# eritpchy/video-subtitle-extractor

Hardware: AMD Instinct MI355X
Metric: OCR frames/sec (det+rec) @1080p (higher is better)
Workload: dtype f16

## Files before the change

include/vse_hip.h:

```cpp
#ifndef VSE_HIP_H
#define VSE_HIP_H

#include <stddef.h>
#include <stdint.h>

#ifdef __cplusplus
extern "C" {
#endif

#define VSE_OK 0
#define VSE_E_INVAL (-1)
#define VSE_E_HIP (-2)
#define VSE_E_UNSUPPORTED (-3)
#define VSE_E_NOMEM (-4)

typedef struct vse_ctx vse_ctx;
typedef struct vse_plan vse_plan;

#pragma pack(push, 1)
typedef struct vse_view {
    int64_t off;
    int32_t arena;
    int32_t n, h, w;
    int32_t c;
// ... 37 lines not shown
                    int64_t frame_stride, int dst_h, int dst_w, int raw_input, void* d_in_f16, float* d_prob, void* stream);
int vse_rec_forward(vse_ctx* ctx, vse_plan* rec_plan, void* ws, const void* d_rec_in_f16, const int32_t* d_widths, int out_level,
                    void* d_idx_maxp, int b, int t, int32_t* d_out_idx, int32_t* d_out_len, float* d_out_conf, void* stream);

typedef struct vse_graph vse_graph;
int vse_rec_graph_create(vse_ctx* ctx, vse_plan* rec_plan, void* ws, const void* d_rec_in_f16, const int32_t* d_widths, int out_level,
                         void* d_idx_maxp, int b, int t, int32_t* d_out_idx, int32_t* d_out_len, float* d_out_conf, void* stream,
                         vse_graph** graph);
int vse_graph_launch(vse_graph* graph, void* stream);
void vse_graph_destroy(vse_graph* graph);

int vse_plan_profile(vse_plan* plan, void* ws, void* const* ext, int n_ext, const int32_t* d_widths, void* stream, float* ms);

const char* vse_op_kernel_name(const vse_op* op);

int vse_det_preprocess(vse_ctx* ctx, const void* d_bgr, int n, int src_h, int src_w, int64_t pitch,
                       int64_t frame_stride, void* d_out_f16, int dst_h, int dst_w, const float* mean3,
                       const float* std3, void* stream);

typedef struct vse_db_params {
    double box_thresh;
    double unclip_ratio;
    float thresh;
    int max_candidates;
    int min_size;
} vse_db_params;

typedef struct vse_box {
    float pts[4][2];
    float score;
// ... 53 lines not shown
```

video-subtitle-extractor_amd/csrc/conv_c3.hip:

```cpp
#include "conv_common.h"
#ifdef VSE_TRACE
#include <stdio.h>
#include <vector>
#define TR_STAMP(i) do { if (tid == 0) tr[i] = __builtin_amdgcn_s_memtime(); } while (0)
#else
#define TR_STAMP(i) do { } while (0)
#endif

#define C3RING 4

template <int RW, int CW, int BN>
__device__ __forceinline__ void conv_c3_body(const ConvParams& p) {
    constexpr int TN = BN / 32;
    constexpr int TH = 2 * RW, TW = 32 * CW;
    constexpr int PW = TW + 8, PH = TH + 2;
    constexpr int PPIX = (PH * PW + 31) / 32 * 32;
    constexpr int PINSTR = PPIX / 32;
    constexpr int PNPL = (PINSTR + 7) / 8;
    constexpr int WROWS = 3 * BN;
    constexpr int WINSTR = WROWS / 32;
    constexpr int PATCH_HALFS = PPIX * 16, WSTAGE_HALFS = WROWS * 16;
    constexpr int PATCH_BYTES = PATCH_HALFS * 2, WSTAGE_BYTES = WSTAGE_HALFS * 2;
    constexpr int ROWB = PW * 32;
    static_assert(RW * CW == 8 && (PW / 8) % 2 == 1, "tile shapes");
    static_assert(2 * PATCH_BYTES + C3RING * WSTAGE_BYTES + 1024 + 4 * BN <= 81920, "two blocks per CU");
    __shared__ __attribute__((aligned(16))) half_t lds[2 * PATCH_HALFS + C3RING * WSTAGE_HALFS + 512 + 2 * BN];
// ... 12 lines not shown
#endif
    TR_STAMP(0);

    unsigned t = xcd_block(blockIdx.x, gridDim.x);
    const int nt = t % p.ntn;  t /= p.ntn;
    const int tx = t % p.tiles_w;  t /= p.tiles_w;
    const int ty = t % p.tiles_h;
    const int oy0 = ty * TH, ox0 = tx * TW, n0 = nt * BN;
    const ConvPackTile pk = conv_pack_tile(p, (int)(t / p.tiles_h), ox0, TW, 3);
    if (ox0 >= pk.vw) return;
    if (conv_tile_right_of_sample<TH, TW>(p, pk.img0, oy0, ox0, n0, BN)) return;
    const int nch1 = p.cinp >> 4;
    const int nchunks = (p.flags & F_HILO) ? 2 * nch1 : nch1;

    int poff[PNPL];
#pragma unroll
    for (int j = 0; j < PNPL; ++j) {
        const int q = 32 * (wave + 8 * j) + (lane >> 1);
        const int kh_ = (lane & 1) ^ ((q >> 3) & 1);
        const int py = q / PW, px = q - py * PW;
        const int iy = oy0 - 1 + py;
        int g, ix;
        const bool ok = conv_pack_src(p, pk, px, g, ix) && (py < PH) && (iy >= 0) && (iy < p.H);
        const long o = (((long)g * p.Hs + (iy >> p.inshift)) * p.Ws + (ix >> p.inshift)) * (long)p.in_ld + kh_ * 8;
        poff[j] = ok ? (int)o : -1;
    }
    const half_t* const in_img = p.in + pk.img0 * (long)p.Hs * p.Ws * p.in_ld;
    const half_t* wptr;
    bool wok;
    const int wnp = p.wnp;
    const int winc = 3 * wnp * 16;
    {
        const int row = 32 * wave + (lane >> 1);
        const int kh_ = (lane & 1) ^ ((row >> 3) & 1);
        const int dy = row / BN, r = row - dy * BN;
        wok = (row < WROWS) && (n0 + r < wnp);
        wptr = wok ? p.w + ((long)dy * wnp + n0 + r) * 16 + kh_ * 8 : p.zero;
    }
    auto issue_patch = [&](int cc) {
        half_t* base = patch0 + (cc & 1) * PATCH_HALFS;
        const bool live = cc < nchunks;
#pragma unroll
        for (int j = 0; j < PNPL; ++j) {
            const int i = wave + 8 * j;
            const half_t* src = (live && poff[j] >= 0) ? in_img + poff[j] + (cc >= nch1 ? cc - nch1 : cc) * 16 : p.zero;
            half_t* dst = base + i * 512;
            if (i >= PINSTR) { src = p.zero; dst = dummy0; }
            glds16_asm(src, dst);
        }
    };
    auto issue_w = [&](int s) {
        half_t* st = ring0 + (s & (C3RING - 1)) * WSTAGE_HALFS;
        glds16_asm(wptr, wave < WINSTR ? st + wave * 512 : dummy0);
        wptr += wok ? winc : 0;
    };

// ... 144 lines not shown
    }
#ifdef VSE_TRACE
    asm volatile("s_waitcnt vmcnt(0)" ::: "memory");
    if (tid == 0 && p.trace) {
        tr[3] = __builtin_amdgcn_s_memtime();
        tr[4] = t_sync;
        for (int i = 0; i < 8; ++i) p.trace[(unsigned long long)blockIdx.x * 8 + i] = tr[i];
    }
#endif
}

template <int RW, int CW>
__global__ __launch_bounds__(512, 4) void conv_c3_kernel(const ConvParams p) { conv_c3_body<RW, CW, C3BN>(p); }
template <int RW, int CW>
__global__ __launch_bounds__(512, 4) void conv_c3n32_kernel(const ConvParams p) { conv_c3_body<RW, CW, 32>(p); }

static const ConvInst kC3Inst[] = {
    CONV_INST(8, 1, 0, conv_c3n32_kernel<8, 1>), CONV_INST(4, 1, 0, conv_c3n32_kernel<4, 2>), CONV_INST(2, 1, 0, conv_c3n32_kernel<2, 4>),
    CONV_INST(8, 0, 0, conv_c3_kernel<8, 1>),    CONV_INST(4, 0, 0, conv_c3_kernel<4, 2>),    CONV_INST(2, 0, 0, conv_c3_kernel<2, 4>),
};

static int launch_conv_c3(const ConvParams& pin, const ConvKernel& k, hipStream_t st) {
    const ConvInst* inst = conv_inst(conv_c3_family(), k);
    if (!inst) return VSE_E_UNSUPPORTED;
    ConvParams p = pin;
    const int rw = k.arg[0], cw = 8 / rw;
    conv_pack_plan(p, 32 * cw, 6);
    if ((double)p.pack_g * p.Hs * p.Ws * p.in_ld > 2.0e9) conv_pack_plan(p, 32 * cw, -1);
    if ((double)p.Hs * p.Ws * p.in_ld > 2.0e9) return VSE_E_UNSUPPORTED;
    const bool hlsum = (p.flags & F_HLSUM) != 0;
    if (hlsum && (p.Np > 32 || (p.flags & F_HILO))) return VSE_E_INVAL;
    const int bn = k.arg[1] ? 32 : C3BN;
    p.wnp = hlsum ? 64 : p.Np;
    p.ntn = hlsum ? 1u : (unsigned)((p.Np + bn - 1) / bn);
    p.tiles_h = (p.OH + 2 * rw - 1) / (2 * rw);
    const unsigned long long blocks = (unsigned long long)((p.nimg + p.pack_g - 1) / p.pack_g) * p.tiles_h * p.tiles_w * p.ntn;
    if (blocks == 0 || blocks > 0x7fffffffull) return VSE_E_INVAL;
    const dim3 grid((unsigned)blocks), block(512);
#ifdef VSE_TRACE
    static unsigned long long* trace_dev = nullptr;
    static size_t trace_cap = 0;
    if (trace_cap < blocks * 8) {
        if (trace_dev) (void)hipFree(trace_dev);
        (void)hipMalloc(&trace_dev, blocks * 8 * sizeof(unsigned long long));
        trace_cap = blocks * 8;
// ... 26 lines not shown
```

video-subtitle-extractor_amd/csrc/conv_common.h:

```cpp
#pragma once
#include "common.h"

#define PTW 32
#define CTW 32
#define CPW 48
#define C3BN 64
#define PW_MAXN 256
#define PW_MAXN_HILO 128
#define DWPW_ROWS_MAX_KS 3
#define DWPW_ROWS_MAX_KS_S1 3

struct ConvParams {
    const half_t* in;
    const half_t* w;
    const float* bias;
    const half_t* res;
    const half_t* zero;
    void* out;
    int H, W, Hs, Ws, in_ld, cinp, inshift;
    int OH, OW;
    long M;
    int kh, kw, sh, sw, ph, pw;
    int Np, nk;
    int nkh;
// ... 18 lines not shown
    const int* wl_out;
    int in_lo_off;
    int res_lo_off;
    int lo_off;
    const half_t* ogate;
    int ogate_ld;
    int wnp;
    const uint8_t* u8src;
    int u8_h, u8_w;
    long u8_pitch, u8_fstride;
    int pack_g, nimg;
    unsigned pack_mag_ow, pack_mag_d;
    int pool_seg, pool_nseg;
};

typedef const __attribute__((address_space(1))) void* gptr_t;
typedef __attribute__((address_space(3))) void* lptr_t;

__device__ __forceinline__ void glds16(const void* g, half_t* l) {
    __builtin_amdgcn_global_load_lds((gptr_t)g, (lptr_t)l, 16, 0, 0);
}

__device__ __forceinline__ void glds16_asm(const void* g, half_t* l) {
    unsigned keep;
    const unsigned dst = __builtin_amdgcn_readfirstlane((unsigned)(size_t)(lptr_t)l);
    asm volatile("s_mov_b32 %0, m0\n\ts_mov_b32 m0, %2\n\ts_nop 0\n\tglobal_load_lds_dwordx4 %1, off\n\ts_mov_b32 m0, %0"
                 : "=&s"(keep) : "v"(g), "s"(dst) : "memory");
}

#define OOB 0x80000000u
// ... 245 lines not shown

struct GemmCfg { int bm, bn, wm, wn, bk, st; };
constexpr GemmCfg kCfg[] = {{128, 128, 2, 2, 32, 3}, {256, 64, 4, 1, 32, 3}, {256, 32, 4, 1, 32, 3}, {256, 128, 4, 2, 32, 3},
                            {256, 256, 4, 4, 32, 3}, {256, 192, 8, 2, 32, 3}, {256, 256, 4, 4, 64, 2}, {256, 192, 8, 2, 64, 2}};

struct SrcGeom { int h, w; long pitch, fstride; };
ConvParams conv_params(const vse_op& o, const TView& in, const TView& res, const TView& in2, const TView& out, const TView& dot_out,
                       const char* wts, const half_t* zero, const int* wl_out, const uint8_t* u8src, const SrcGeom& src);
ConvKernel conv_select(const ConvParams& p, int Kp);
int conv_kernel_name(const ConvKernel& k, char* buf, size_t n);
int launch_conv(const vse_op& o, const TView& in, const TView& res, const TView& in2, const TView& out, const TView& dot_out,
                const char* wts, const half_t* zero, const int* wl_out, const uint8_t* u8src, const SrcGeom& src, hipStream_t st);
ConvKernel conv_pool_select(const vse_op* ops, int n_ops, int i);
int launch_conv_pool(const vse_op& conv, const ConvKernel& k, const TView& in, const TView& pool_out, const char* wts, const half_t* zero,
                     hipStream_t st);
static inline long conv_images(const ConvParams& p) { return p.OH && p.OW ? p.M / ((long)p.OH * p.OW) : 0; }
int conv_pack_group(long images, int OW, int TW, int spare, int gap);
void conv_pack_plan(ConvParams& p, int TW, int spare);
```

video-subtitle-extractor_amd/csrc/conv_select.hip:

```cpp
#include <stdlib.h>
#include <cstdio>
#include "conv_common.h"


static int conv_gemm_mode(int kh, int kw, int sh, int sw, int ph, int pw, int cinp, int Kp, int inshift, int flags) {
    (void)sh; (void)sw;
    if (inshift || (flags & (F_PATCH | F_DOT1 | F_SRC2))) return 0;
    if (cinp % 32) return 0;
    if (kh * kw > 31) return 0;
    if (kh < 2 * ph + 1 || kw < 2 * pw) return 0;
    if (kh == 1 && kw == 1 && ph == 0 && pw == 0 && Kp == cinp) return 2;
    return 1;
}
static bool conv_gemm_span_ok(const ConvParams& p, int Kp) {
    const double span = ((double)512 * p.sw + (512.0 / p.OW + 3) * p.sh * p.Ws + (double)p.kh * p.Ws + p.kw) * p.in_ld * 2;
    return !(span > 1.9e9 || (double)Kp * p.Np * 2 > 1.9e9);
}

static int conv_gemm_config(int Np, int cinp, long M) {
    auto ntn = [&](int bn) { return (long)((Np + bn - 1) / bn); };
    auto deep = [&](int c) { return cinp % 64 == 0 ? c + 2 : c; };
    if (Np <= 32) return 2;
    if (Np <= 64) return 1;
    const long mt = (M + 255) / 256;
// ... 296 lines not shown
}

int launch_conv_pool(const vse_op& conv, const ConvKernel& k, const TView& in, const TView& pool_out, const char* wts, const half_t* zero,
                     hipStream_t st) {
    if (k.family != CK_C3POOL || !in.ptr || !pool_out.ptr || !zero) return VSE_E_INVAL;
    const TView none{nullptr, 0, 0, 0, 0, 0, 0};
    const TView shape{nullptr, conv.out.n, conv.out.h, conv.out.w, conv.out.c, conv.out.ld, conv.out.esize};
    ConvParams p = conv_params(conv, in, none, none, shape, none, wts, zero, nullptr, nullptr, SrcGeom{0, 0, 0, 0});
    if (in.c != p.cinp || (in.ld & 7)) return VSE_E_INVAL;
    p.out = pool_out.ptr;
    p.out_ld = pool_out.ld;
    return conv_launch(p, k, st);
}


int launch_conv(const vse_op& o, const TView& in, const TView& res, const TView& in2, const TView& out, const TView& dot_out,
                const char* wts, const half_t* zero, const int* wl_out, const uint8_t* u8src, const SrcGeom& src, hipStream_t st) {
    const ConvParams p = conv_params(o, in, res, in2, out, dot_out, wts, zero, wl_out, u8src, src);
    const int f = p.flags, Np = p.Np, cinp = p.cinp;
    if (f & F_SRC2) {
        if (!in2.ptr || in2.esize != 2 || (in2.ld & 7) || in.c + in2.c != cinp) return VSE_E_INVAL;
        if ((in2.h << p.in2_shift) != p.H || (in2.w << p.in2_shift) != p.W) return VSE_E_INVAL;
    } else if (in.c != cinp) {
        return VSE_E_INVAL;
    }
    if (in.esize != 2 || ((in.ld & 7) && !((f & F_UP2HEAD) && in.ld == 1)) || (cinp & 7)) return VSE_E_INVAL;
    if ((f & F_RES) && (res.esize != 2 || (res.ld & 3))) return VSE_E_INVAL;
    if ((!(f & (F_DOT1 | F_ONECH)) && (out.ld & 3)) || (Np & 7)) return VSE_E_INVAL;
    if ((f & F_ONECH) && (!(f & F_PIXSHUF) || !(f & F_OUT_F32) || Np != 32 || out.ld != 1 || out.esize != 4 || (f & F_RES)))
        return VSE_E_INVAL;
// ... 16 lines not shown
```

video-subtitle-extractor_amd/csrc/vse_runtime.hip:

```cpp
#include <stdlib.h>
#include <cstdarg>
#include <cstdio>
#include <cstring>
#include <string>
#include <vector>

#include "conv_common.h"

static thread_local std::string g_err;
static void set_err(const char* fmt, ...) {
    char buf[512];
    va_list ap;
    va_start(ap, fmt);
    vsnprintf(buf, sizeof buf, fmt, ap);
    va_end(ap);
    g_err = buf;
}
void vse_set_error(const char* msg) { g_err = msg ? msg : ""; }
#define HIP_TRY(expr)                                                                  \
    do {                                                                               \
        hipError_t e_ = (expr);                                                        \
        if (e_ != hipSuccess) {                                                        \
            set_err("%s failed: %s (%s:%d)", #expr, hipGetErrorString(e_), __FILE__, __LINE__); \
            return VSE_E_HIP;                                                          \
        }                                                                              \
    } while (0)

struct vse_ctx {
    int device;
    std::vector<void*> weights;
    std::vector<size_t> weight_bytes;
    void* zero_page;
};

struct vse_plan {
    vse_ctx* ctx;
    int weights_id;
    std::vector<vse_op> ops;
    std::vector<ConvKernel> pooled;
    size_t ws_bytes;
    int max_ext;
    int n_levels;
    int batch;
    bool u8_source;
    int src_h, src_w;
    long src_pitch, src_fstride;
};

int vse_frame_change_launch(const void* d_bgr, int n, int64_t pitch, int64_t frame_stride, int y0, int y1, int x0, int x1, int edge_thresh,
                            void* d_state, int reset, int32_t* d_counts, void* stream);
int vse_scene_change_plane_pitch(int aw);
int vse_scene_change_launch(const void* d_bgr, int n, int64_t pitch, int64_t frame_stride, int scale, int ah, int aw, int search, int bias,
                            void* d_state, int reset, void* d_ws, int32_t* d_counts, void* stream);
size_t vse_audio_match_ws(const long* m, const long* n, int nq);
int vse_audio_match_launch(const uint8_t* const* pat, const uint8_t* const* win, const long* m, const long* n, int nq, void* d_ws,
                           unsigned long long* d_out, void* stream);

extern "C" {

const char* vse_last_error(void) { return g_err.c_str(); }
size_t vse_sizeof_op(void) { return sizeof(vse_op); }
size_t vse_sizeof_view(void) { return sizeof(vse_view); }
int vse_abi_version(void) { return 4; }

int vse_init(int device_id, vse_ctx** out) {
    if (!out) return VSE_E_INVAL;
    int count = 0;
    HIP_TRY(hipGetDeviceCount(&count));
    if (device_id < 0 || device_id >= count) {
        set_err("device %d not present (%d visible)", device_id, count);
        return VSE_E_INVAL;
// ... 109 lines not shown
                set_err("op %d: chain descriptor out of the weight blob", i);
                delete p;
                return VSE_E_INVAL;
            }
            if (hdr[0] != 0x43484e31 || hdr[1] != o.p[3] || hdr[2] != o.p[4] || hdr[5] != o.p[2] || hdr[3] < 0 || hdr[4] < 0 ||
                (size_t)o.w_off + (size_t)hdr[4] + (size_t)hdr[3] > wbytes) {
                set_err("op %d: chain descriptor does not match its record (magic %#x, stages %d / %d, buffers %d / %d, LDS %d / %d)", i, hdr[0],
                        hdr[1], o.p[3], hdr[2], o.p[4], hdr[5], o.p[2]);
                delete p;
                return VSE_E_INVAL;
            }
        }
    }
    p->pooled.assign(n_ops, ConvKernel{CK_NONE, VSE_OK, {0, 0, 0}});
    for (int i = 0; i + 1 < n_ops && !p->n_levels; ++i) p->pooled[i] = conv_pool_select(ops, n_ops, i);
    *out = p;
    return VSE_OK;
}

void vse_plan_destroy(vse_plan* p) { delete p; }

static inline TView resolve(const vse_view& v, char* ws, char* wts, void* const* ext) {
    TView t;
    t.ptr = nullptr;
    t.n = v.n; t.h = v.h; t.w = v.w; t.c = v.c; t.ld = v.ld; t.esize = v.esize;
    if (v.n == 0) return t;
    char* base = v.arena == 0 ? ws : (v.arena == 1 ? wts : reinterpret_cast<char*>(ext[v.arena - 2]));
    t.ptr = base + v.off;
    return t;
}

static int run_op(vse_plan* p, int i, char* ws, void* const* ext, const int32_t* wtab, hipStream_t st, const SrcGeom& src) {
    const vse_op& o = p->ops[i];
    const int* wl_in = (wtab && o.p[P_WLIN]) ? wtab + (size_t)(o.p[P_WLIN] - 1) * p->batch : nullptr;
    const int* wl_out = (wtab && o.p[P_WLOUT]) ? wtab + (size_t)(o.p[P_WLOUT] - 1) * p->batch : nullptr;
    char* wts = reinterpret_cast<char*>(p->ctx->weights[p->weights_id]);
    const TView in0 = resolve(o.in0, ws, wts, ext), in1 = resolve(o.in1, ws, wts, ext),
                in2 = resolve(o.in2, ws, wts, ext), out = resolve(o.out, ws, wts, ext),
                out2 = resolve(o.out2, ws, wts, ext);
    int rc;
    if (i > 0 && p->pooled[i - 1].family == CK_C3POOL) return VSE_OK;
    if (p->pooled[i].family == CK_C3POOL) {
        const TView pool_out = resolve(p->ops[i + 1].out, ws, wts, ext);
        rc = launch_conv_pool(o, p->pooled[i], in0, pool_out, wts, reinterpret_cast<const half_t*>(p->ctx->zero_page), st);
    } else if (o.kind == OP_CONV) {
        const uint8_t* u8src = (o.flags & F_U8SRC) ? reinterpret_cast<const uint8_t*>(ext[0]) : nullptr;
        rc = launch_conv(o, in0, in1, in2, out, out2, wts, reinterpret_cast<const half_t*>(p->ctx->zero_page), wl_out, u8src, src, st);
    } else if (o.kind == OP_CHAIN) {
        rc = launch_chain(o, in0, out, out2, in2, wts, st);
    } else {
        rc = launch_simple_op(o, in0, in1, in2, out, out2, wts, wl_in, wl_out, st);
    }
    if (rc != VSE_OK) set_err("op %d (kind %d) failed to launch: rc=%d (%s)", i, o.kind, rc, hipGetErrorString(hipGetLastError()));
    return rc;
}

static int check_run(vse_plan* p, void* ws, void* const* ext, int n_ext, const int32_t* d_widths, const char* who) {
// ... 288 lines not shown
    if (rc0 != VSE_OK) return rc0;
    hipStream_t st = reinterpret_cast<hipStream_t>(stream);
    const int n = (int)p->ops.size();
    std::vector<hipEvent_t> ev(n + 1);
    for (auto& e : ev) HIP_TRY(hipEventCreate(&e));
    HIP_TRY(hipEventRecord(ev[0], st));
    for (int i = 0; i < n; ++i) {
        int rc = run_op(p, i, reinterpret_cast<char*>(ws), ext, d_widths, st, SrcGeom{p->src_h, p->src_w, p->src_pitch, p->src_fstride});
        if (rc != VSE_OK) return rc;
        HIP_TRY(hipEventRecord(ev[i + 1], st));
    }
    HIP_TRY(hipStreamSynchronize(st));
    for (int i = 0; i < n; ++i) HIP_TRY(hipEventElapsedTime(&ms[i], ev[i], ev[i + 1]));
    for (int i = 1; i < n; ++i)
        if (p->pooled[i - 1].family == CK_C3POOL) ms[i] = 0.f;
    for (auto& e : ev) (void)hipEventDestroy(e);
    return VSE_OK;
}

}
```

video-subtitle-extractor_amd/engine.py:

```python
import ctypes as C
import os

import numpy as np

from . import compiler, ir

_HERE = os.path.dirname(os.path.abspath(__file__))
LIB_PATH = os.environ.get("VSE_LIB_PATH") or os.path.join(_HERE, "libvse_hip.so")

EXPORTS = [
    "vse_init", "vse_destroy", "vse_last_error", "vse_sizeof_op", "vse_sizeof_view", "vse_abi_version",
    "vse_weights_upload", "vse_weights_free", "vse_plan_create", "vse_plan_destroy", "vse_plan_run", "vse_plan_run_ragged",
    "vse_plan_width_levels", "vse_plan_profile", "vse_op_kernel_name", "vse_det_preprocess", "vse_db_workspace_bytes",
    "vse_db_postprocess", "vse_rec_preprocess", "vse_rec_preprocess_scratch_bytes", "vse_ctc_collapse", "vse_ctc_collapse_ragged",
    "vse_det_forward", "vse_rec_forward", "vse_plan_set_source", "vse_plan_takes_frames",
    "vse_rec_graph_create", "vse_graph_launch", "vse_graph_destroy", "vse_frame_change_state_bytes", "vse_frame_change",
    "vse_audio_match_workspace_bytes", "vse_audio_match", "vse_scene_change_state_bytes", "vse_scene_change_workspace_bytes",
    "vse_scene_change",
]


class VseError(RuntimeError):
    pass


class DbParams(C.Structure):
    _fields_ = [("box_thresh", C.c_double), ("unclip_ratio", C.c_double), ("thresh", C.c_float),
                ("max_candidates", C.c_int), ("min_size", C.c_int)]


class Box(C.Structure):
    _fields_ = [("pts", C.c_float * 2 * 4), ("score", C.c_float), ("frame", C.c_int)]

# ... 45 lines not shown
    lib.vse_rec_graph_create.argtypes = [C.c_void_p, C.c_void_p, C.c_void_p, C.c_void_p, C.c_void_p, C.c_int, C.c_void_p, C.c_int, C.c_int,
                                         C.c_void_p, C.c_void_p, C.c_void_p, C.c_void_p, C.POINTER(C.c_void_p)]
    lib.vse_graph_launch.argtypes = [C.c_void_p, C.c_void_p]
    lib.vse_graph_destroy.argtypes = [C.c_void_p]
    lib.vse_graph_destroy.restype = None
    lib.vse_plan_set_source.argtypes = [C.c_void_p, C.c_int, C.c_int, C.c_int64, C.c_int64]
    lib.vse_plan_takes_frames.argtypes = [C.c_void_p]
    lib.vse_det_forward.argtypes = [C.c_void_p, C.c_void_p, C.c_void_p, C.c_void_p, C.c_int, C.c_int, C.c_int, C.c_int64, C.c_int64,
                                    C.c_int, C.c_int, C.c_int, C.c_void_p, C.c_void_p, C.c_void_p]
    lib.vse_rec_forward.argtypes = [C.c_void_p, C.c_void_p, C.c_void_p, C.c_void_p, C.c_void_p, C.c_int, C.c_void_p, C.c_int, C.c_int,
                                    C.c_void_p, C.c_void_p, C.c_void_p, C.c_void_p]
    lib.vse_plan_profile.argtypes = [C.c_void_p, C.c_void_p, C.POINTER(C.c_void_p), C.c_int, C.c_void_p, C.c_void_p,
                                     C.POINTER(C.c_float)]
    lib.vse_op_kernel_name.argtypes = [C.c_void_p]
    lib.vse_op_kernel_name.restype = C.c_char_p
    lib.vse_det_preprocess.argtypes = [C.c_void_p, C.c_void_p, C.c_int, C.c_int, C.c_int, C.c_int64, C.c_int64,
                                       C.c_void_p, C.c_int, C.c_int, C.POINTER(C.c_float), C.POINTER(C.c_float),
                                       C.c_void_p]
    lib.vse_db_postprocess.argtypes = [C.c_void_p, C.c_void_p, C.c_int, C.c_int, C.c_int, C.c_int, C.c_int,
                                       C.POINTER(DbParams), C.c_void_p, C.c_size_t, C.POINTER(Box), C.c_int,
                                       C.POINTER(C.c_int), C.c_void_p]
    lib.vse_rec_preprocess.argtypes = [C.c_void_p, C.c_void_p, C.c_int, C.c_int, C.c_int, C.c_int64, C.c_int64,
                                       C.POINTER(Crop), C.c_int, C.c_void_p, C.c_int, C.c_int, C.c_void_p,
                                       C.c_size_t, C.c_void_p]
    lib.vse_ctc_collapse.argtypes = [C.c_void_p, C.c_void_p, C.c_int, C.c_int, C.c_void_p, C.c_void_p, C.c_void_p,
                                     C.c_void_p]
    lib.vse_ctc_collapse_ragged.argtypes = [C.c_void_p, C.c_void_p, C.c_int, C.c_int, C.c_void_p, C.c_void_p, C.c_void_p,
                                            C.c_void_p, C.c_void_p]
    lib.vse_frame_change_state_bytes.restype = C.c_size_t
    lib.vse_frame_change_state_bytes.argtypes = [C.c_int, C.c_int]
# ... 4 lines not shown
    lib.vse_audio_match.argtypes = [C.c_void_p, C.c_void_p, C.c_int64, C.c_void_p, C.c_int64, C.c_void_p, C.c_int, C.c_void_p,
                                    C.c_size_t, C.c_void_p, C.c_void_p]
    lib.vse_scene_change_state_bytes.restype = C.c_size_t
    lib.vse_scene_change_state_bytes.argtypes = [C.c_int, C.c_int, C.c_int]
    lib.vse_scene_change_workspace_bytes.restype = C.c_size_t
    lib.vse_scene_change_workspace_bytes.argtypes = [C.c_int, C.c_int, C.c_int, C.c_int]
    lib.vse_scene_change.argtypes = [C.c_void_p, C.c_void_p, C.c_int, C.c_int, C.c_int, C.c_int64, C.c_int64, C.c_int, C.c_int, C.c_int,
                                     C.c_void_p, C.c_int, C.c_void_p, C.c_size_t, C.c_void_p, C.c_void_p]
    if lib.vse_sizeof_op() != ir.OP_DT.itemsize or lib.vse_sizeof_view() != ir.VIEW_DT.itemsize:
        raise VseError(f"ABI mismatch: vse_op {lib.vse_sizeof_op()} vs {ir.OP_DT.itemsize}, "
                       f"vse_view {lib.vse_sizeof_view()} vs {ir.VIEW_DT.itemsize}")
    _lib = lib
    return lib


def op_kernel_names(ops):
    lib = load_library()
    ops = np.ascontiguousarray(ops)
    base = ops.ctypes.data
    return [lib.vse_op_kernel_name(C.c_void_p(base + i * ops.itemsize)).decode() for i in range(len(ops))]


def profiled_kernel_names(ops, ms):
    names = op_kernel_names(ops)
    for i in range(1, len(names)):
        if (int(ops[i]["kind"]) == ir.OP_POOL and int(ops[i - 1]["kind"]) == ir.OP_CONV and float(ms[i]) == 0.0
                and names[i - 1].startswith("conv_patch_kernel<")):
            names[i - 1] = "conv_c3pool_kernel<%s>" % names[i - 1].split(",")[1].strip()
    return names


def _check(rc, what):
    if rc < 0:
        raise VseError(f"{what} failed (rc={rc}): {load_library().vse_last_error().decode(errors='replace')}")
    return rc


def _torch():
    import torch
    if not torch.cuda.is_available():
        raise VseError("no HIP device visible: the OCR hot path runs only on MI355X (gfx950); no CPU fallback")
    return torch


# ... 389 lines not shown
    def profile_frames(self, frames_u8, dst_h, dst_w, slot=0):
        if not self.fuse_preprocess:
            return self.profile(self.ctx.det_preprocess(frames_u8, dst_h, dst_w, raw=self.input_norm is not None), slot)
        t = self.ctx.torch
        n, h, w, _ = frames_u8.shape
        self.program(n, dst_h, dst_w)
        prog, handle = self._ensure((n, dst_h, dst_w))
        _check(self.ctx.lib.vse_plan_set_source(handle, h, w, frames_u8.stride(1), frames_u8.stride(0)), "vse_plan_set_source")
        outs = [t.empty((o["n"], o["h"], o["w"], o["ld"]), dtype=t.float32, device=self.ctx.tdev) for o in prog.outputs]
        ptrs = (C.c_void_p * (1 + len(outs)))(frames_u8.data_ptr(), *[o.data_ptr() for o in outs])
        ms = (C.c_float * len(prog.ops))()
        ws = self._workspace((n, dst_h, dst_w), prog, slot)
        self.last_outs = outs
        _check(self.ctx.lib.vse_plan_profile(handle, C.c_void_p(ws.data_ptr()), ptrs, len(ptrs), None, self.ctx.stream(), ms),
               "vse_plan_profile")
        names = profiled_kernel_names(prog.ops, ms)
        return np.array(ms[:], dtype=np.float32), prog, names

    def rec_forward(self, x, widths=None, slot=0):
        t = self.ctx.torch
        assert x.dtype == t.float16 and x.is_contiguous() and x.shape[3] == 8
        n, h, w, _ = x.shape
        self.program(n, h, w)
        prog, handle = self._ensure((n, h, w))
        assert len(prog.outputs) == 1 and prog.outputs[0]["kind"] == "idx_maxp"
        tt = prog.outputs[0]["w"]
        wt = self._width_table(prog, widths, n, w)
        idx_maxp = t.empty((n, 1, tt, 2), dtype=t.float32, device=self.ctx.tdev)
        oi = t.zeros((n, tt), dtype=t.int32, device=self.ctx.tdev)
        ol = t.empty((n,), dtype=t.int32, device=self.ctx.tdev)
        oc = t.empty((n,), dtype=t.float32, device=self.ctx.tdev)
# ... 41 lines not shown
        return bufs["oi"].clone(), bufs["ol"].clone(), bufs["oc"].clone()

    def profile(self, x, slot=0, widths=None):
        n, h, w, _ = x.shape
        self.program(n, h, w)
        prog, handle = self._ensure((n, h, w))
        outs, ptrs = self._ext(prog, x)
        ms = (C.c_float * len(prog.ops))()
        ws = self._workspace((n, h, w), prog, slot)
        wt = self._width_table(prog, widths, n, w)
        self.last_tlen = wt[prog.out_level] if wt is not None else None
        self.last_outs = outs
        _check(self.ctx.lib.vse_plan_profile(handle, C.c_void_p(ws.data_ptr()), ptrs, len(ptrs),
                                             C.c_void_p(wt.data_ptr()) if wt is not None else None, self.ctx.stream(), ms),
               "vse_plan_profile")
        variants = profiled_kernel_names(prog.ops, ms)
        return np.array(ms[:], dtype=np.float32), prog, variants
```

Measured before the change: 2097.

## Fuse channel-concat resizes into 3x3 conv via multi-part gather input table

Adds a gather variant of the c3 3x3 conv kernel that reads its input channels from up to four source tensors (with per-part upsample shift), driven by a small device-side part table. The plan detects convs whose input is a concat written by resize ops and absorbs those resizes, skipping their launches and the intermediate concat write and read. When a source would be overwritten before the conv, the resize is kept as a plain copy. The cost is extra per-chunk part switching and address recomputation inside the conv, plus extra plan analysis logic.

```diff
diff --git a/include/vse_hip.h b/include/vse_hip.h
--- a/include/vse_hip.h
+++ b/include/vse_hip.h
@@ -75,6 +75,10 @@
 
 const char* vse_op_kernel_name(const vse_op* op);
 
+const char* vse_plan_kernel_name(vse_plan* plan, int i);
+int vse_plan_set_concat_gather(vse_plan* plan, int mode);
+int vse_concat_gather_parts(const vse_op* ops, int n_ops, int i, int32_t* info);
+
 int vse_det_preprocess(vse_ctx* ctx, const void* d_bgr, int n, int src_h, int src_w, int64_t pitch,
                        int64_t frame_stride, void* d_out_f16, int dst_h, int dst_w, const float* mean3,
                        const float* std3, void* stream);
diff --git a/video-subtitle-extractor_amd/csrc/conv_c3.hip b/video-subtitle-extractor_amd/csrc/conv_c3.hip
--- a/video-subtitle-extractor_amd/csrc/conv_c3.hip
+++ b/video-subtitle-extractor_amd/csrc/conv_c3.hip
@@ -9,7 +9,7 @@
 
 #define C3RING 4
 
-template <int RW, int CW, int BN>
+template <int RW, int CW, int BN, bool GATHER = false>
 __device__ __forceinline__ void conv_c3_body(const ConvParams& p) {
     constexpr int TN = BN / 32;
     constexpr int TH = 2 * RW, TW = 32 * CW;
@@ -52,18 +52,47 @@
     const int nchunks = (p.flags & F_HILO) ? 2 * nch1 : nch1;
 
     int poff[PNPL];
-#pragma unroll
-    for (int j = 0; j < PNPL; ++j) {
-        const int q = 32 * (wave + 8 * j) + (lane >> 1);
-        const int kh_ = (lane & 1) ^ ((q >> 3) & 1);
-        const int py = q / PW, px = q - py * PW;
-        const int iy = oy0 - 1 + py;
-        int g, ix;
-        const bool ok = conv_pack_src(p, pk, px, g, ix) && (py < PH) && (iy >= 0) && (iy < p.H);
-        const long o = (((long)g * p.Hs + (iy >> p.inshift)) * p.Ws + (ix >> p.inshift)) * (long)p.in_ld + kh_ * 8;
-        poff[j] = ok ? (int)o : -1;
-    }
-    const half_t* const in_img = p.in + pk.img0 * (long)p.Hs * p.Ws * p.in_ld;
+    const half_t* in_img;
+    int part_i = 0, part_next = 0x7fffffff;
+    auto load_part = [&](int pi) __attribute__((always_inline)) {
+        typedef const __attribute__((address_space(4))) ConvPart* cpart_t;
+        const cpart_t tab = reinterpret_cast<cpart_t>(reinterpret_cast<uintptr_t>(p.in2));
+        pi = __builtin_amdgcn_readfirstlane(pi);
+        ConvPart e;
+        e.off = tab[pi].off; e.ld = tab[pi].ld; e.shift = tab[pi].shift; e.c0 = tab[pi].c0; e.h = tab[pi].h; e.w = tab[pi].w;
+        part_i = pi;
+        part_next = pi + 1 < p.in2_ld ? tab[pi + 1].c0 >> 4 : 0x7fffffff;
+        in_img = p.in + e.off + pk.img0 * (long)e.h * e.w * e.ld - e.c0;
+        int ln = lane;
+        asm volatile("" : "+v"(ln));
+#pragma unroll
+        for (int j = 0; j < PNPL; ++j) {
+            const int q = 32 * (wave + 8 * j) + (ln >> 1);
+            const int kh_ = (ln & 1) ^ ((q >> 3) & 1);
+            const int py = q / PW, px = q - py * PW;
+            const int iy = oy0 - 1 + py;
+            int g, ix;
+            const bool ok = conv_pack_src(p, pk, px, g, ix) && (py < PH) && (iy >= 0) && (iy < p.H);
+            const long o = (((long)g * e.h + (iy >> e.shift)) * e.w + (ix >> e.shift)) * (long)e.ld + kh_ * 8;
+            poff[j] = ok ? (int)o : -1;
+        }
+    };
+    if constexpr (GATHER) {
+        load_part(0);
+    } else {
+#pragma unroll
+        for (int j = 0; j < PNPL; ++j) {
+            const int q = 32 * (wave + 8 * j) + (lane >> 1);
+            const int kh_ = (lane & 1) ^ ((q >> 3) & 1);
+            const int py = q / PW, px = q - py * PW;
+            const int iy = oy0 - 1 + py;
+            int g, ix;
+            const bool ok = conv_pack_src(p, pk, px, g, ix) && (py < PH) && (iy >= 0) && (iy < p.H);
+            const long o = (((long)g * p.Hs + (iy >> p.inshift)) * p.Ws + (ix >> p.inshift)) * (long)p.in_ld + kh_ * 8;
+            poff[j] = ok ? (int)o : -1;
+        }
+        in_img = p.in + pk.img0 * (long)p.Hs * p.Ws * p.in_ld;
+    }
     const half_t* wptr;
     bool wok;
     const int wnp = p.wnp;
@@ -78,6 +107,9 @@
     auto issue_patch = [&](int cc) {
         half_t* base = patch0 + (cc & 1) * PATCH_HALFS;
         const bool live = cc < nchunks;
+        if constexpr (GATHER) {
+            if (cc == part_next) load_part(part_i + 1);
+        }
 #pragma unroll
         for (int j = 0; j < PNPL; ++j) {
             const int i = wave + 8 * j;
@@ -252,10 +284,17 @@
 __global__ __launch_bounds__(512, 4) void conv_c3_kernel(const ConvParams p) { conv_c3_body<RW, CW, C3BN>(p); }
 template <int RW, int CW>
 __global__ __launch_bounds__(512, 4) void conv_c3n32_kernel(const ConvParams p) { conv_c3_body<RW, CW, 32>(p); }
+template <int RW, int CW>
+__global__ __launch_bounds__(512, 4) void conv_c3_gather_kernel(const ConvParams p) { conv_c3_body<RW, CW, C3BN, true>(p); }
+template <int RW, int CW>
+__global__ __launch_bounds__(512, 4) void conv_c3n32_gather_kernel(const ConvParams p) { conv_c3_body<RW, CW, 32, true>(p); }
 
 static const ConvInst kC3Inst[] = {
     CONV_INST(8, 1, 0, conv_c3n32_kernel<8, 1>), CONV_INST(4, 1, 0, conv_c3n32_kernel<4, 2>), CONV_INST(2, 1, 0, conv_c3n32_kernel<2, 4>),
     CONV_INST(8, 0, 0, conv_c3_kernel<8, 1>),    CONV_INST(4, 0, 0, conv_c3_kernel<4, 2>),    CONV_INST(2, 0, 0, conv_c3_kernel<2, 4>),
+    CONV_INST(8, 1, 1, conv_c3n32_gather_kernel<8, 1>), CONV_INST(4, 1, 1, conv_c3n32_gather_kernel<4, 2>),
+    CONV_INST(2, 1, 1, conv_c3n32_gather_kernel<2, 4>), CONV_INST(8, 0, 1, conv_c3_gather_kernel<8, 1>),
+    CONV_INST(4, 0, 1, conv_c3_gather_kernel<4, 2>),    CONV_INST(2, 0, 1, conv_c3_gather_kernel<2, 4>),
 };
 
 static int launch_conv_c3(const ConvParams& pin, const ConvKernel& k, hipStream_t st) {
@@ -267,6 +306,8 @@
     if ((double)p.pack_g * p.Hs * p.Ws * p.in_ld > 2.0e9) conv_pack_plan(p, 32 * cw, -1);
     if ((double)p.Hs * p.Ws * p.in_ld > 2.0e9) return VSE_E_UNSUPPORTED;
     const bool hlsum = (p.flags & F_HLSUM) != 0;
+    if (k.arg[2] && (!p.in2 || p.in2_ld < 1 || p.in2_ld > CONV_MAX_PARTS || p.inshift || p.wl_out || (p.flags & (F_HILO | F_HLSUM | F_SRC2))))
+        return VSE_E_INVAL;
     if (hlsum && (p.Np > 32 || (p.flags & F_HILO))) return VSE_E_INVAL;
     const int bn = k.arg[1] ? 32 : C3BN;
     p.wnp = hlsum ? 64 : p.Np;
diff --git a/video-subtitle-extractor_amd/csrc/conv_common.h b/video-subtitle-extractor_amd/csrc/conv_common.h
--- a/video-subtitle-extractor_amd/csrc/conv_common.h
+++ b/video-subtitle-extractor_amd/csrc/conv_common.h
@@ -56,6 +56,12 @@
     int pool_seg, pool_nseg;
 };
 
+#define CONV_MAX_PARTS 4
+struct ConvPart {
+    long off;
+    int ld, shift, c0, h, w, pad_;
+};
+
 typedef const __attribute__((address_space(1))) void* gptr_t;
 typedef __attribute__((address_space(3))) void* lptr_t;
 
@@ -331,6 +337,21 @@
 ConvKernel conv_pool_select(const vse_op* ops, int n_ops, int i);
 int launch_conv_pool(const vse_op& conv, const ConvKernel& k, const TView& in, const TView& pool_out, const char* wts, const half_t* zero,
                      hipStream_t st);
+struct ConvConcat {
+    int nparts;
+    struct {
+        vse_view src;
+        vse_view copy_from;
+        int shift, c0;
+        int writer;
+        int absorbed;
+    } part[CONV_MAX_PARTS];
+};
+ConvKernel conv_concat_select(const vse_op* ops, int n_ops, int i, ConvConcat* cc = nullptr);
+void conv_concat_table(const vse_op& conv, const ConvConcat& cc, ConvPart* tab);
+void conv_concat_force_copy(const vse_op& conv, ConvConcat& cc);
+int launch_conv_gather(const vse_op& conv, const ConvKernel& k, const TView& in, const TView& res, const TView& out, const char* wts,
+                       const half_t* zero, const ConvPart* d_tab, int nparts, hipStream_t st);
 static inline long conv_images(const ConvParams& p) { return p.OH && p.OW ? p.M / ((long)p.OH * p.OW) : 0; }
 int conv_pack_group(long images, int OW, int TW, int spare, int gap);
 void conv_pack_plan(ConvParams& p, int TW, int spare);
diff --git a/video-subtitle-extractor_amd/csrc/conv_select.hip b/video-subtitle-extractor_amd/csrc/conv_select.hip
--- a/video-subtitle-extractor_amd/csrc/conv_select.hip
+++ b/video-subtitle-extractor_amd/csrc/conv_select.hip
@@ -334,6 +334,137 @@
 }
 
 
+static bool channel_slice(const vse_view& w, const vse_view& v, int* c0) {
+    if (w.n == 0 || w.arena != v.arena || w.n != v.n || w.h != v.h || w.w != v.w || w.ld != v.ld || w.esize != v.esize) return false;
+    const int64_t d = w.off - v.off;
+    if (d < 0 || d % v.esize || d / v.esize + w.c > v.c) return false;
+    *c0 = (int)(d / v.esize);
+    return true;
+}
+static bool touches(const vse_op& o, const vse_view& v) {
+    return views_overlap(o.in0, v) || views_overlap(o.in1, v) || views_overlap(o.in2, v) || views_overlap(o.out, v) || views_overlap(o.out2, v);
+}
+static bool reads(const vse_op& o, const vse_view& v) {
+    return views_overlap(o.in0, v) || views_overlap(o.in1, v) || (o.kind != OP_CHAIN && views_overlap(o.in2, v)) ||
+           (o.kind != OP_CONV && o.kind != OP_CHAIN && views_overlap(o.out2, v));
+}
+static bool writes(const vse_op& o, const vse_view& v) {
+    return views_overlap(o.out, v) || ((o.kind == OP_CONV || o.kind == OP_CHAIN) && views_overlap(o.out2, v)) ||
+           (o.kind == OP_CHAIN && views_overlap(o.in2, v));
+}
+static void part_to_copy(const vse_view& V, ConvConcat& t, int q) {
+    auto& e = t.part[q];
+    if (!e.absorbed || e.copy_from.n) return;
+    e.copy_from = e.src;
+    e.src.off = V.off + (int64_t)e.c0 * V.esize;
+    e.src.arena = V.arena;
+    e.src.ld = V.ld;
+}
+void conv_concat_force_copy(const vse_op& conv, ConvConcat& cc) {
+    for (int q = 0; q < cc.nparts; ++q) part_to_copy(conv.in0, cc, q);
+}
+
+ConvKernel conv_concat_select(const vse_op* ops, int n_ops, int i, ConvConcat* cc) {
+    const ConvKernel no{CK_NONE, VSE_OK, {0, 0, 0}};
+    if (!ops || i < 1 || i >= n_ops) return no;
+    const vse_op& c = ops[i];
+    if (c.kind != OP_CONV || (c.flags & ~(F_COL | F_RES)) || !(c.flags & F_COL)) return no;
+    if (c.p[P_KH] != 3 || c.p[P_KW] != 3 || c.p[P_SH] != 1 || c.p[P_SW] != 1 || c.p[P_PH] != 1 || c.p[P_PW] != 1) return no;
+    if (c.p[P_INSHIFT] || c.p[P_LO_OUT] || c.p[P_LO_RES] || c.p[P_WLIN] || c.p[P_WLOUT] || c.in2.n || c.out2.n) return no;
+    const vse_view& V = c.in0;
+    if (V.n == 0 || V.arena != 0 || V.esize != 2 || V.c != c.p[P_CINP] || (V.ld & 7) || (V.off & 15)) return no;
+    auto shape = [](const vse_view& v) { return TView{nullptr, v.n, v.h, v.w, v.c, v.ld, v.esize}; };
+    const ConvParams prm = conv_params(c, shape(c.in0), shape(c.in1), shape(c.in2), shape(c.out), shape(c.out2), nullptr, nullptr, nullptr, nullptr,
+                                       SrcGeom{0, 0, 0, 0});
+    const ConvKernel k = conv_select(prm, c.p[P_KTOT]);
+    if (k.family != CK_C3 || k.rc != VSE_OK || k.arg[2]) return no;
+
+    ConvConcat t{};
+    int covered = 0, first = i;
+    auto add = [&](const vse_view& src, const vse_view& from, int shift, int c0, int ch, int writer) {
+        if (t.nparts == CONV_MAX_PARTS || (c0 & 15) || (ch & 15) || ch <= 0) return false;
+        for (int q = 0; q < t.nparts; ++q)
+            if (c0 < t.part[q].c0 + t.part[q].src.c && t.part[q].c0 < c0 + ch) return false;
+        auto& e = t.part[t.nparts++];
+        e.src = src; e.src.c = ch; e.copy_from = from; e.shift = shift; e.c0 = c0; e.writer = writer;
+        covered += ch;
+        return true;
+    };
+    auto source_ok = [&](const vse_view& sv, int shift, int ch) {
+        return sv.n == V.n && sv.arena == 0 && sv.esize == 2 && sv.c >= ch && !(sv.ld & 7) && !(sv.off & 15) && shift >= 0 && shift <= 3 &&
+               (sv.h << shift) == V.h && (sv.w << shift) == V.w && !views_overlap(sv, V);
+    };
+    for (int j = i - 1; j >= 0 && covered < V.c; --j) {
+        const vse_op& o = ops[j];
+        int c0;
+        if (!channel_slice(o.out, V, &c0)) {
+            if (touches(o, V)) return no;
+            continue;
+        }
+        if (views_overlap(o.in0, V) || views_overlap(o.in1, V) || views_overlap(o.in2, V) || views_overlap(o.out2, V)) return no;
+        if (o.p[P_WLIN] || o.p[P_WLOUT]) return no;
+        first = j;
+        if (o.kind == OP_CONV) {
+            if (o.p[P_LO_OUT] || (o.flags & (F_PIXSHUF | F_OUT_F32 | F_DOT1 | F_ONECH)) || o.out.c != o.p[P_COUT]) return no;
+            if (!add(o.out, vse_view{}, 0, c0, o.out.c, j)) return no;
+        } else if (o.kind == OP_RESIZE && !(o.flags & F_GATE) && !(o.flags & ~(F_SRC2 | F_RES))) {
+            const bool two = (o.flags & F_SRC2) != 0;
+            const int ca = two ? o.in0.c : o.out.c, cb = two ? o.in2.c : 0;
+            if (o.in1.n || o.out2.n || (!two && o.in2.n) || ca + cb != o.out.c) return no;
+            if (!source_ok(o.in0, o.p[0], ca) || !add(o.in0, vse_view{}, o.p[0], c0, ca, j)) return no;
+            if (two && (!source_ok(o.in2, o.p[1], cb) || !add(o.in2, vse_view{}, o.p[1], c0 + ca, cb, j))) return no;
+        } else {
+            return no;
+        }
+    }
+    if (covered != V.c || t.nparts < 2) return no;
+    bool any = false;
+    for (int q = 0; q < t.nparts; ++q) any = any || ops[t.part[q].writer].kind == OP_RESIZE;
+    if (!any) return no;
+    (void)first;
+    for (int j = i + 1; j < n_ops; ++j) {
+        const vse_op& o = ops[j];
+        if (reads(o, V)) return no;
+        if (writes(o, V)) break;
+    }
+    for (int a = 0; a < t.nparts; ++a)
+        for (int b = a + 1; b < t.nparts; ++b)
+            if (t.part[b].c0 < t.part[a].c0) { const auto x = t.part[a]; t.part[a] = t.part[b]; t.part[b] = x; }
+    for (int q = 0; q < t.nparts; ++q) {
+        auto& e = t.part[q];
+        if (ops[e.writer].kind != OP_RESIZE) continue;
+        e.absorbed = 1;
+        bool lives = !views_overlap(c.out, e.src) && !views_overlap(c.out2, e.src);
+        for (int j = e.writer + 1; j < i && lives; ++j) lives = !writes(ops[j], e.src);
+        if (!lives) part_to_copy(V, t, q);
+    }
+    for (int q = 0; q < t.nparts; ++q)
+        if (16.0 * t.part[q].src.h * t.part[q].src.w * (t.part[q].src.ld > V.ld ? t.part[q].src.ld : V.ld) > 2.0e9) return no;
+    if (cc) *cc = t;
+    return ConvKernel{CK_C3, VSE_OK, {k.arg[0], k.arg[1], 1}};
+}
+
+void conv_concat_table(const vse_op& conv, const ConvConcat& cc, ConvPart* tab) {
+    for (int q = 0; q < cc.nparts; ++q) {
+        const auto& e = cc.part[q];
+        tab[q] = ConvPart{(e.src.off - conv.in0.off) / 2, e.src.ld, e.shift, e.c0, e.src.h, e.src.w, 0};
+    }
+}
+
+int launch_conv_gather(const vse_op& conv, const ConvKernel& k, const TView& in, const TView& res, const TView& out, const char* wts,
+                       const half_t* zero, const ConvPart* d_tab, int nparts, hipStream_t st) {
+    if (k.family != CK_C3 || !k.arg[2] || !in.ptr || !out.ptr || !zero || !d_tab) return VSE_E_INVAL;
+    const TView none{nullptr, 0, 0, 0, 0, 0, 0};
+    ConvParams p = conv_params(conv, in, res, none, out, none, wts, zero, nullptr, nullptr, SrcGeom{0, 0, 0, 0});
+    if (in.c != p.cinp || in.esize != 2 || (in.ld & 7) || (p.cinp & 15) || (out.ld & 3) || (p.Np & 7)) return VSE_E_INVAL;
+    if ((p.flags & F_RES) && (res.esize != 2 || (res.ld & 3))) return VSE_E_INVAL;
+    if (out.h != p.OH || out.w != p.OW || out.n != in.n) return VSE_E_INVAL;
+    p.in2 = reinterpret_cast<const half_t*>(d_tab);
+    p.in2_ld = nparts;
+    return conv_launch(p, k, st);
+}
+
+
 int launch_conv(const vse_op& o, const TView& in, const TView& res, const TView& in2, const TView& out, const TView& dot_out,
                 const char* wts, const half_t* zero, const int* wl_out, const uint8_t* u8src, const SrcGeom& src, hipStream_t st) {
     const ConvParams p = conv_params(o, in, res, in2, out, dot_out, wts, zero, wl_out, u8src, src);
diff --git a/video-subtitle-extractor_amd/csrc/vse_runtime.hip b/video-subtitle-extractor_amd/csrc/vse_runtime.hip
--- a/video-subtitle-extractor_amd/csrc/vse_runtime.hip
+++ b/video-subtitle-extractor_amd/csrc/vse_runtime.hip
@@ -38,6 +38,12 @@
     int weights_id;
     std::vector<vse_op> ops;
     std::vector<ConvKernel> pooled;
+    std::vector<ConvKernel> gathered;
+    std::vector<ConvConcat> parts;
+    std::vector<int> gather_slot;
+    std::vector<char> absorbed;
+    std::vector<std::vector<std::pair<vse_view, vse_view>>> copies;
+    ConvPart* d_parts;
     size_t ws_bytes;
     int max_ext;
     int n_levels;
@@ -55,6 +61,8 @@
 size_t vse_audio_match_ws(const long* m, const long* n, int nq);
 int vse_audio_match_launch(const uint8_t* const* pat, const uint8_t* const* win, const long* m, const long* n, int nq, void* d_ws,
                            unsigned long long* d_out, void* stream);
+
+static int plan_concat_commit(vse_plan* p);
 
 extern "C" {
 
@@ -194,11 +202,97 @@
     }
     p->pooled.assign(n_ops, ConvKernel{CK_NONE, VSE_OK, {0, 0, 0}});
     for (int i = 0; i + 1 < n_ops && !p->n_levels; ++i) p->pooled[i] = conv_pool_select(ops, n_ops, i);
+    p->gathered.assign(n_ops, ConvKernel{CK_NONE, VSE_OK, {0, 0, 0}});
+    p->parts.assign(n_ops, ConvConcat{});
+    p->gather_slot.assign(n_ops, -1);
+    p->absorbed.assign(n_ops, 0);
+    p->copies.assign(n_ops, {});
+    p->d_parts = nullptr;
+    for (int i = 0; i < n_ops && !p->n_levels; ++i) {
+        ConvConcat cc;
+        const ConvKernel k = conv_concat_select(ops, n_ops, i, &cc);
+        if (k.family != CK_C3) continue;
+        bool taken = false;
+        for (int j = 0; j < i; ++j)
+            for (int q = 0; q < cc.nparts && p->gathered[j].family == CK_C3; ++q)
+                for (int r = 0; r < p->parts[j].nparts; ++r) taken = taken || (cc.part[q].absorbed && p->parts[j].part[r].writer == cc.part[q].writer);
+        if (taken) continue;
+        p->gathered[i] = k;
+        p->parts[i] = cc;
+    }
+    if (plan_concat_commit(p) != VSE_OK) {
+        if (p->d_parts) (void)hipFree(p->d_parts);
+        delete p;
+        return VSE_E_HIP;
+    }
     *out = p;
     return VSE_OK;
 }
 
-void vse_plan_destroy(vse_plan* p) { delete p; }
+void vse_plan_destroy(vse_plan* p) {
+    if (p && p->d_parts) (void)hipFree(p->d_parts);
+    delete p;
+}
+
+static int plan_concat_commit(vse_plan* p) {
+    const int n = (int)p->ops.size();
+    p->absorbed.assign(n, 0);
+    p->copies.assign(n, {});
+    std::vector<ConvPart> tabs;
+    for (int i = 0; i < n; ++i) {
+        p->gather_slot[i] = -1;
+        if (p->gathered[i].family != CK_C3) continue;
+        p->gather_slot[i] = (int)tabs.size() / CONV_MAX_PARTS;
+        tabs.resize(tabs.size() + CONV_MAX_PARTS, ConvPart{});
+        conv_concat_table(p->ops[i], p->parts[i], &tabs[tabs.size() - CONV_MAX_PARTS]);
+        for (int q = 0; q < p->parts[i].nparts; ++q) {
+            const auto& e = p->parts[i].part[q];
+            if (!e.absorbed) continue;
+            p->absorbed[e.writer] = 1;
+            if (e.copy_from.n) p->copies[e.writer].push_back({e.copy_from, e.src});
+        }
+    }
+    if (tabs.empty()) return VSE_OK;
+    HIP_TRY(hipSetDevice(p->ctx->device));
+    if (!p->d_parts) HIP_TRY(hipMalloc(&p->d_parts, tabs.size() * sizeof(ConvPart)));
+    HIP_TRY(hipMemcpy(p->d_parts, tabs.data(), tabs.size() * sizeof(ConvPart), hipMemcpyHostToDevice));
+    return VSE_OK;
+}
+
+int vse_plan_set_concat_gather(vse_plan* p, int mode) {
+    if (!p || (mode != 0 && mode != 2)) return VSE_E_INVAL;
+    for (size_t i = 0; i < p->ops.size(); ++i) {
+        if (p->gathered[i].family != CK_C3) continue;
+        if (mode == 0) p->gathered[i] = ConvKernel{CK_NONE, VSE_OK, {0, 0, 0}};
+        else conv_concat_force_copy(p->ops[i], p->parts[i]);
+    }
+    return plan_concat_commit(p);
+}
+
+int vse_concat_gather_parts(const vse_op* ops, int n_ops, int i, int32_t* info) {
+    if (!ops || n_ops <= 0) return VSE_E_INVAL;
+    for (int j = 0; j < n_ops; ++j)
+        if (ops[j].p[P_WLIN] > 0 || ops[j].p[P_WLOUT] > 0) return 0;
+    ConvConcat cc{};
+    if (conv_concat_select(ops, n_ops, i, &cc).family != CK_C3) return 0;
+    for (int q = 0; q < cc.nparts && info; ++q) {
+        const auto& e = cc.part[q];
+        info[4 * q] = e.c0; info[4 * q + 1] = e.src.c; info[4 * q + 2] = e.shift; info[4 * q + 3] = !e.absorbed ? 0 : (e.copy_from.n ? 2 : 1);
+    }
+    return cc.nparts;
+}
+
+const char* vse_plan_kernel_name(vse_plan* p, int i) {
+    static thread_local char buf[96];
+    buf[0] = 0;
+    if (!p || i < 0 || i >= (int)p->ops.size()) return buf;
+    if (i > 0 && p->pooled[i - 1].family == CK_C3POOL) return buf;
+    if (p->pooled[i].family == CK_C3POOL) conv_kernel_name(p->pooled[i], buf, sizeof buf);
+    else if (p->gathered[i].family == CK_C3) conv_kernel_name(p->gathered[i], buf, sizeof buf);
+    else if (p->absorbed[i]) snprintf(buf, sizeof buf, "%s", p->copies[i].empty() ? "" : "resize_kernel");
+    else return vse_op_kernel_name(&p->ops[i]);
+    return buf;
+}
 
 static inline TView resolve(const vse_view& v, char* ws, char* wts, void* const* ext) {
     TView t;
@@ -220,7 +314,24 @@
                 out2 = resolve(o.out2, ws, wts, ext);
     int rc;
     if (i > 0 && p->pooled[i - 1].family == CK_C3POOL) return VSE_OK;
-    if (p->pooled[i].family == CK_C3POOL) {
+    if (p->absorbed[i]) {
+        vse_op cp{};
+        cp.kind = OP_RESIZE;
+        const TView none{nullptr, 0, 0, 0, 0, 0, 0};
+        for (const auto& ft : p->copies[i]) {
+            const TView from = resolve(ft.first, ws, wts, ext), to = resolve(ft.second, ws, wts, ext);
+            rc = launch_simple_op(cp, from, none, none, to, none, wts, nullptr, nullptr, st);
+            if (rc != VSE_OK) {
+                set_err("op %d (absorbed resize) failed to launch: rc=%d (%s)", i, rc, hipGetErrorString(hipGetLastError()));
+                return rc;
+            }
+        }
+        return VSE_OK;
+    }
+    if (p->gathered[i].family == CK_C3) {
+        rc = launch_conv_gather(o, p->gathered[i], in0, in1, out, wts, reinterpret_cast<const half_t*>(p->ctx->zero_page),
+                                p->d_parts + (size_t)CONV_MAX_PARTS * p->gather_slot[i], p->parts[i].nparts, st);
+    } else if (p->pooled[i].family == CK_C3POOL) {
         const TView pool_out = resolve(p->ops[i + 1].out, ws, wts, ext);
         rc = launch_conv_pool(o, p->pooled[i], in0, pool_out, wts, reinterpret_cast<const half_t*>(p->ctx->zero_page), st);
     } else if (o.kind == OP_CONV) {
@@ -539,6 +650,8 @@
     for (int i = 0; i < n; ++i) HIP_TRY(hipEventElapsedTime(&ms[i], ev[i], ev[i + 1]));
     for (int i = 1; i < n; ++i)
         if (p->pooled[i - 1].family == CK_C3POOL) ms[i] = 0.f;
+    for (int i = 0; i < n; ++i)
+        if (p->absorbed[i] && p->copies[i].empty()) ms[i] = 0.f;
     for (auto& e : ev) (void)hipEventDestroy(e);
     return VSE_OK;
 }
diff --git a/video-subtitle-extractor_amd/engine.py b/video-subtitle-extractor_amd/engine.py
--- a/video-subtitle-extractor_amd/engine.py
+++ b/video-subtitle-extractor_amd/engine.py
@@ -16,7 +16,8 @@
     "vse_det_forward", "vse_rec_forward", "vse_plan_set_source", "vse_plan_takes_frames",
     "vse_rec_graph_create", "vse_graph_launch", "vse_graph_destroy", "vse_frame_change_state_bytes", "vse_frame_change",
     "vse_audio_match_workspace_bytes", "vse_audio_match", "vse_scene_change_state_bytes", "vse_scene_change_workspace_bytes",
-    "vse_scene_change",
+    "vse_scene_change", "vse_plan_kernel_name", "vse_plan_set_concat_gather",
+    "vse_concat_gather_parts",
 ]
 
 
@@ -92,6 +93,10 @@
                                      C.POINTER(C.c_float)]
     lib.vse_op_kernel_name.argtypes = [C.c_void_p]
     lib.vse_op_kernel_name.restype = C.c_char_p
+    lib.vse_plan_kernel_name.argtypes = [C.c_void_p, C.c_int]
+    lib.vse_plan_kernel_name.restype = C.c_char_p
+    lib.vse_plan_set_concat_gather.argtypes = [C.c_void_p, C.c_int]
+    lib.vse_concat_gather_parts.argtypes = [C.c_void_p, C.c_int, C.c_int, C.c_void_p]
     lib.vse_det_preprocess.argtypes = [C.c_void_p, C.c_void_p, C.c_int, C.c_int, C.c_int, C.c_int64, C.c_int64,
                                        C.c_void_p, C.c_int, C.c_int, C.POINTER(C.c_float), C.POINTER(C.c_float),
                                        C.c_void_p]
@@ -126,20 +131,22 @@
     return lib
 
 
-def op_kernel_names(ops):
+def op_kernel_names(ops, plan=None):
     lib = load_library()
+    if plan is not None:
+        return [lib.vse_plan_kernel_name(plan, i).decode() for i in range(len(ops))]
     ops = np.ascontiguousarray(ops)
     base = ops.ctypes.data
     return [lib.vse_op_kernel_name(C.c_void_p(base + i * ops.itemsize)).decode() for i in range(len(ops))]
 
 
-def profiled_kernel_names(ops, ms):
-    names = op_kernel_names(ops)
-    for i in range(1, len(names)):
-        if (int(ops[i]["kind"]) == ir.OP_POOL and int(ops[i - 1]["kind"]) == ir.OP_CONV and float(ms[i]) == 0.0
-                and names[i - 1].startswith("conv_patch_kernel<")):
-            names[i - 1] = "conv_c3pool_kernel<%s>" % names[i - 1].split(",")[1].strip()
-    return names
+def concat_gather_parts(ops, i):
+    lib = load_library()
+    ops = np.ascontiguousarray(ops)
+    info = np.zeros(16, np.int32)
+    n = lib.vse_concat_gather_parts(ops.ctypes.data_as(C.c_void_p), len(ops), i, info.ctypes.data_as(C.c_void_p))
+    _check(n, "vse_concat_gather_parts")
+    return [(int(info[4 * q]), int(info[4 * q + 1]), int(info[4 * q + 2]), ("direct", "source", "copy")[info[4 * q + 3]]) for q in range(n)]
 
 
 def _check(rc, what):
@@ -559,7 +566,7 @@
         self.last_outs = outs
         _check(self.ctx.lib.vse_plan_profile(handle, C.c_void_p(ws.data_ptr()), ptrs, len(ptrs), None, self.ctx.stream(), ms),
                "vse_plan_profile")
-        names = profiled_kernel_names(prog.ops, ms)
+        names = op_kernel_names(prog.ops, handle)
         return np.array(ms[:], dtype=np.float32), prog, names
 
     def rec_forward(self, x, widths=None, slot=0):
@@ -631,5 +638,5 @@
         _check(self.ctx.lib.vse_plan_profile(handle, C.c_void_p(ws.data_ptr()), ptrs, len(ptrs),
                                              C.c_void_p(wt.data_ptr()) if wt is not None else None, self.ctx.stream(), ms),
                "vse_plan_profile")
-        variants = profiled_kernel_names(prog.ops, ms)
+        variants = op_kernel_names(prog.ops, handle)
         return np.array(ms[:], dtype=np.float32), prog, variants
```

Result: no change. 2116 (median of 6 runs) (+0.9%).
